# awentzonline/tartangan

Measured on AMD Instinct MI355X. Metric: images/sec (G+D step), higher is better.
Workload: dtype f32; 1 GPU; 128:3 SA-GAN cnn G+D step (R1 penalty, Adam x2, EMA), 128x128 RGB, batch 64/GPU, global batch 64; trainer=cnn, gan_config=128:3, global_batch=64, parallelism=dp1, hip_graphs=True

## Files before the change

tartangan_amd/csrc/conv.hip:

```cpp
#include <cstdlib>
#include <type_traits>
#include <utility>

#include "common.h"

namespace {

typedef float f32x16 __attribute__((ext_vector_type(16)));
typedef float f32x4 __attribute__((ext_vector_type(4)));

constexpr int CT_THREADS = 256;

template <int TH_, int TW_, int NI_>
struct Geo {
  static constexpr int TH = TH_, TW = TW_, NI = NI_, NPIX = TH_ * TW_ * NI_;
  static_assert(NPIX == 512 || NPIX == 256 || NPIX == 64, "a pixel tile is 512 / 256 pixels (waves split pixels) or 64 (waves split K)");
  static constexpr int PPW = (NPIX == 64) ? 64 : NPIX / 4;
  static_assert(TW_ % 4 == 0, "rows are staged as float4");
};
using G4 = Geo<4, 4, 16>;
using G8 = Geo<8, 8, 4>;
using G16 = Geo<16, 16, 1>;
using GX = Geo<8, 32, 1>;
using G4k = Geo<4, 4, 4>;
// ... 623 lines not shown
  auto advance = [&]() {
    xb += xstep; xbytes -= xstep;
    wb += wstep; wbytes -= wstep;
  };
  auto issue = [&](int c0, float* buf) {
    const __amdgpu_buffer_rsrc_t rx = __builtin_amdgcn_make_buffer_rsrc(const_cast<char*>(xb), 0, (int)xbytes, 0x00020000);
    const __amdgpu_buffer_rsrc_t rw = __builtin_amdgcn_make_buffer_rsrc(const_cast<char*>(wb), 0, (int)wbytes, 0x00020000);
    const int cvalid = s.Cin - c0;
#pragma unroll
    for (int i = 0; i < NPIECE; ++i) issue_piece(i, buf, rx, rw, cvalid);
    advance();
  };

  int lane_b[NT];
#pragma unroll
  for (int n = 0; n < NT; ++n) lane_b[n] = (h + g0 * KG) * P::CIS + P::pix(pix0 + n * MF + j);
  const int lane_a = DGRAD ? ((h + g0 * KG) * F::RS + j * 9 + 8) : (j * F::RS + (h + g0 * KG) * 9);

  typename Core::acc_t acc[MT][NT];
  Core::zero(acc);

#ifdef TG_DIAG_STAMPS
  asm volatile("" :: "v"(poff[0]), "v"(woff[0]), "v"(lane_b[0]), "v"(lane_a));
  const uint64_t st_setup = __builtin_amdgcn_s_memtime();
#endif
  if (DB) issue(0, lds);
  int buf = 0;
#ifdef TG_DIAG_STAMPS
  const uint64_t st_c0 = __builtin_amdgcn_s_memtime(), st_r0 = __builtin_amdgcn_s_memrealtime();
  uint64_t st_wait = 0, st_bar = 0, st_issue = 0, st_mfma = 0, st_prev = 0, st_last = 0;
#endif
  for (int c0 = 0; c0 < s.Cin; c0 += CK) {
    if constexpr (!DB) {
      __syncthreads();
      issue(c0, lds);
    }
#ifdef TG_DIAG_STAMPS
    const uint64_t ph0 = __builtin_amdgcn_s_memtime();
#endif
    asm volatile("s_waitcnt vmcnt(0)" ::: "memory");
#ifdef TG_DIAG_STAMPS
    const uint64_t ph1 = __builtin_amdgcn_s_memtime();
#endif
    __syncthreads();
#ifdef TG_DIAG_STAMPS
    const uint64_t ph2 = __builtin_amdgcn_s_memtime();
#endif
    if constexpr (DB) {
      if (c0 + CK < s.Cin) issue(c0 + CK, lds + (buf ^ 1) * BUF);
    }
#ifdef TG_DIAG_STAMPS
    const uint64_t ph3 = __builtin_amdgcn_s_memtime();
    st_wait += ph1 - ph0; st_bar += ph2 - ph1; st_issue += ph3 - ph2; st_last = ph3;
    if (c0 > 0) st_mfma += ph0 - st_prev;
    st_prev = ph3;
#endif
    const float* pl = lds + buf * BUF;
    const float* wl = pl + PBUF;
#ifdef TG_DIAG_STAMPS
    if (xcd_swizzle & 4) { buf ^= 1; continue; }
#endif
    if (prio) __builtin_amdgcn_s_setprio(0);
#pragma unroll
    for (int gi = 0; gi < NG / (WK ? 4 : 1); ++gi) {
      const int g = gi * (WK ? 4 : 1);
#pragma unroll
      for (int tap = 0; tap < 9; ++tap) {
        const int kh = tap / 3, kw = tap % 3;
        float a[MT], b[NT];
#pragma unroll
        for (int m = 0; m < MT; ++m)
          a[m] = DGRAD ? wl[lane_a + (g * KG) * F::RS + m * MF * 9 - tap] : wl[lane_a + m * MF * F::RS + (g * KG) * 9 + tap];
#pragma unroll
        for (int n = 0; n < NT; ++n) b[n] = pl[lane_b[n] + (g * KG) * P::CIS + kh * P::PWS + kw];
#pragma unroll
        for (int m = 0; m < MT; ++m)
#pragma unroll
          for (int n = 0; n < NT; ++n) {
            if constexpr (MF == 32)
              acc[m][n] = __builtin_amdgcn_mfma_f32_32x32x2f32(a[m], b[n], acc[m][n], 0, 0, 0);
            else
              acc[m][n] = __builtin_amdgcn_mfma_f32_16x16x4f32(a[m], b[n], acc[m][n], 0, 0, 0);
          }
      }
    }
    if (prio) __builtin_amdgcn_s_setprio(3);
    if (DB) buf ^= 1;
  }
#ifdef TG_DIAG_STAMPS
  {
    const uint64_t st_c1 = __builtin_amdgcn_s_memtime(), st_r1 = __builtin_amdgcn_s_memrealtime();
    const int slot = blockIdx.y * gridDim.x + blockIdx.x;
    if (threadIdx.x == 0 && slot < TG_DIAG_SLOTS) { tg_diag_stamps[2 * slot] = st_c1 - st_c0; tg_diag_stamps[2 * slot + 1] = st_r1 - st_r0; }
    st_mfma += st_c1 - st_last;
    if (lane == 0 && slot < TG_DIAG_SLOTS) {
      unsigned long long* ph = tg_diag_phases + (slot * 4 + wave) * 4;
      ph[0] = st_wait; ph[1] = st_bar; ph[2] = st_issue; ph[3] = st_mfma;
    }
  }
#endif
  if constexpr (WK) {
    __syncthreads();
    float* red = lds;
#pragma unroll
    for (int m = 0; m < MT; ++m)
#pragma unroll
      for (int n = 0; n < NT; ++n)
#pragma unroll
        for (int r = 0; r < NREG; ++r) red[(((wave * MT + m) * NT + n) * NREG + r) * 64 + lane] = acc[m][n][r];
    __syncthreads();
    constexpr int PW_ = MT * NT * NREG * 64;
#pragma unroll
    for (int m = 0; m < MT; ++m)
#pragma unroll
      for (int n = 0; n < NT; ++n)
#pragma unroll
        for (int r = 0; r < NREG; ++r) {
          const int e = ((m * NT + n) * NREG + r) * 64 + lane;
          acc[m][n][r] = (red[e] + red[PW_ + e]) + (red[2 * PW_ + e] + red[3 * PW_ + e]);
        }
  }
#ifdef TG_DIAG_STAMPS
  if ((xcd_swizzle & 2) && acc[0][0][0] != 12345.678f) return;
#endif
  Core::epilogue(acc, bias, residual, y, s, tc, co0, pix0, j, h, wave);
#ifdef TG_DIAG_STAMPS
  {
    const uint64_t e0 = __builtin_amdgcn_s_memtime();
    asm volatile("s_waitcnt vmcnt(0)" ::: "memory");
    const uint64_t e1 = __builtin_amdgcn_s_memtime();
    const int slot = blockIdx.y * gridDim.x + blockIdx.x;
    if (lane == 0 && slot < TG_DIAG_SLOTS) {
      unsigned long long* ph = tg_diag_life + (slot * 4 + wave) * 4;
      ph[0] = st_c0 - st_begin; ph[1] = e0 - st_c0; ph[2] = e1 - e0; ph[3] = st_setup - st_begin;
    }
  }
#endif
}

template <int CO, int PX>
__global__ void __launch_bounds__(256)
conv1x1_direct_kernel(const float* __restrict__ x, const float* __restrict__ w, const float* __restrict__ bias,
                      const float* __restrict__ residual, float* __restrict__ y, int Cin, int Cout, int HW, int w_so, int w_si) {
  __shared__ __attribute__((aligned(16))) float wl[1024];
  for (int e = threadIdx.x; e < Cin * CO; e += 256) {
    const int ci = e / CO, co = e - ci * CO;
    wl[e] = co < Cout ? w[co * w_so + ci * w_si] : 0.f;
  }
  __syncthreads();
  const int b = blockIdx.y;
  const int p = (blockIdx.x * 256 + threadIdx.x) * PX;
  if (p >= HW) return;
  const float* xb = x + (int64_t)b * Cin * HW + p;
  float acc[CO][PX];
#pragma unroll
  for (int co = 0; co < CO; ++co)
#pragma unroll
    for (int u = 0; u < PX; ++u) acc[co][u] = 0.f;
#pragma unroll 4
  for (int ci = 0; ci < Cin; ++ci) {
    float xv[PX];
    if (PX == 4) {
      const float4 t = *reinterpret_cast<const float4*>(xb + (int64_t)ci * HW);
      xv[0] = t.x; xv[1] = t.y; xv[2] = t.z; xv[3] = t.w;
    } else {
      xv[0] = xb[(int64_t)ci * HW];
    }
#pragma unroll
    for (int c4 = 0; c4 < CO / 4; ++c4) {
      const float4 wv = *reinterpret_cast<const float4*>(&wl[ci * CO + 4 * c4]);
      const float ww[4] = {wv.x, wv.y, wv.z, wv.w};
#pragma unroll
      for (int k = 0; k < 4; ++k)
#pragma unroll
        for (int u = 0; u < PX; ++u) acc[4 * c4 + k][u] = fmaf(ww[k], xv[u], acc[4 * c4 + k][u]);
    }
  }
  const int64_t ob = (int64_t)b * Cout * HW + p;
#pragma unroll
  for (int co = 0; co < CO; ++co) {
    if (co >= Cout) break;
    const float bv = bias ? bias[co] : 0.f;
    float o[PX];
#pragma unroll
    for (int u = 0; u < PX; ++u) o[u] = acc[co][u] + bv;
    const int64_t off = ob + (int64_t)co * HW;
    if (PX == 4) {
      if (residual) {
        const float4 r = *reinterpret_cast<const float4*>(residual + off);
        o[0] += r.x; o[1] += r.y; o[2] += r.z; o[3] += r.w;
      }
      *reinterpret_cast<float4*>(y + off) = make_float4(o[0], o[1], o[2], o[3]);
    } else {
      if (residual) o[0] += residual[off];
      y[off] = o[0];
    }
  }
}

template <int CO>
static int launch_conv1x1_direct(const float* x, const float* w, const float* bias, const float* residual, float* y, Shape s,
                                 bool dgrad, hipStream_t st) {
  const int HW = s.H * s.W;
  const int w_so = dgrad ? 1 : s.Cin, w_si = dgrad ? s.Cout : 1;
  const bool vec = (HW % 4 == 0) && tg_aligned16(x) && tg_aligned16(y) && (!residual || tg_aligned16(residual));
  if (vec) {
    dim3 grid((HW / 4 + 255) / 256, s.B);
    conv1x1_direct_kernel<CO, 4><<<grid, 256, 0, st>>>(x, w, bias, residual, y, s.Cin, s.Cout, HW, w_so, w_si);
  } else {
    dim3 grid((HW + 255) / 256, s.B);
    conv1x1_direct_kernel<CO, 1><<<grid, 256, 0, st>>>(x, w, bias, residual, y, s.Cin, s.Cout, HW, w_so, w_si);
  }
  return tg_launch_status();
}
static inline int conv1x1_co(int Cout) { return Cout <= 4 ? 4 : 8; }
static inline bool conv1x1_direct_ok(const Shape& s) { return s.Cout <= 8 && s.Cin * conv1x1_co(s.Cout) <= 1024 && s.B <= 65535; }
static int launch_conv1x1(const float* x, const float* w, const float* bias, const float* residual, float* y, Shape s, bool dgrad,
                          hipStream_t st) {
  if (s.Cout <= 4) return launch_conv1x1_direct<4>(x, w, bias, residual, y, s, dgrad, st);
  return launch_conv1x1_direct<8>(x, w, bias, residual, y, s, dgrad, st);
}

struct ChanSegs {
  float* p[3];
  int start[4];
  __device__ __forceinline__ int find(int c) const { return c >= start[2] ? 2 : (c >= start[1] ? 1 : 0); }
  __device__ __forceinline__ int width(int k) const { return start[k + 1] - start[k]; }
};
static inline ChanSegs one_seg(const float* p, int channels) {
  ChanSegs g;
  g.p[0] = g.p[1] = g.p[2] = const_cast<float*>(p);
  g.start[0] = 0; g.start[1] = g.start[2] = g.start[3] = channels;
  return g;
}
static inline ChanSegs three_segs(const float* p0, const float* p1, const float* p2, int c0, int c1, int c2) {
  ChanSegs g;
  g.p[0] = const_cast<float*>(p0); g.p[1] = const_cast<float*>(p1); g.p[2] = const_cast<float*>(p2);
  g.start[0] = 0; g.start[1] = c0; g.start[2] = c0 + c1; g.start[3] = c0 + c1 + c2;
  return g;
}

template <int NCO>
__global__ void __launch_bounds__(256)
conv1x1_mfma_kernel(ChanSegs xs, const float* __restrict__ w, const float* __restrict__ bias,
                    const float* __restrict__ residual, ChanSegs ys, int Cin, int Cout, int HW, int64_t quads,
                    int w_so, int w_si) {
  const int lane = threadIdx.x & 63, j = lane & 15, h = lane >> 4;
  const int64_t q = ((int64_t)blockIdx.x * 4 + (threadIdx.x >> 6)) * 16 + j;
  const bool live = q < quads;
  const int qpp = HW >> 2;
  const int64_t b = live ? q / qpp : 0;
  const int p = live ? (int)(q - b * qpp) * 4 : 0;
  f32x4 acc[NCO][4];
#pragma unroll
  for (int m = 0; m < NCO; ++m)
#pragma unroll
    for (int r = 0; r < 4; ++r) acc[m][r] = f32x4{0.f, 0.f, 0.f, 0.f};
  int wrow[NCO];
#pragma unroll
  for (int m = 0; m < NCO; ++m) wrow[m] = min(16 * m + j, Cout - 1) * w_so;
  constexpr int U = 4;
  for (int k0 = 0; k0 < Cin; k0 += 4 * U) {
    float4 xv[U];
    float a[U][NCO];
#pragma unroll
    for (int u = 0; u < U; ++u) {
      const int ci = k0 + 4 * u + h;
      const bool ok = live && ci < Cin;
      const int cc = min(ci, Cin - 1);
      const int k = xs.find(cc);
      const float* src = xs.p[k] + ((b * xs.width(k) + (cc - xs.start[k])) * HW + p);
      xv[u] = ok ? *reinterpret_cast<const float4*>(src) : make_float4(0.f, 0.f, 0.f, 0.f);
#pragma unroll
      for (int m = 0; m < NCO; ++m) a[u][m] = (ci < Cin) ? w[wrow[m] + cc * w_si] : 0.f;
    }
#pragma unroll
    for (int u = 0; u < U; ++u) {
      const float bx[4] = {xv[u].x, xv[u].y, xv[u].z, xv[u].w};
#pragma unroll
      for (int m = 0; m < NCO; ++m)
#pragma unroll
        for (int r = 0; r < 4; ++r) acc[m][r] = __builtin_amdgcn_mfma_f32_16x16x4f32(a[u][m], bx[r], acc[m][r], 0, 0, 0);
    }
  }
  if (!live) return;
  const float* rb = residual ? residual + (b * Cout) * HW + p : nullptr;
#pragma unroll
  for (int m = 0; m < NCO; ++m)
#pragma unroll
    for (int i = 0; i < 4; ++i) {
      const int co = 16 * m + 4 * h + i;
      if (co >= Cout) continue;
      const float bv = bias ? bias[co] : 0.f;
      float4 o = make_float4(acc[m][0][i] + bv, acc[m][1][i] + bv, acc[m][2][i] + bv, acc[m][3][i] + bv);
      if (rb) {
        const float4 t = *reinterpret_cast<const float4*>(rb + (int64_t)co * HW);
        o.x += t.x; o.y += t.y; o.z += t.z; o.w += t.w;
      }
      const int k = ys.find(co);
      *reinterpret_cast<float4*>(ys.p[k] + ((b * ys.width(k) + (co - ys.start[k])) * HW + p)) = o;
    }
}

static inline bool conv1x1_mfma_ok(const float* x, const float* residual, const float* y, const Shape& s) {
  return (s.H * s.W) % 4 == 0 && s.Cout <= 128 && tg_aligned16(x) && tg_aligned16(y) && (!residual || tg_aligned16(residual));
}
static int launch_conv1x1_segs(ChanSegs xs, const float* w, const float* bias, const float* residual, ChanSegs ys, Shape s, bool dgrad,
                               hipStream_t st) {
  const int HW = s.H * s.W;
  const int64_t quads = (int64_t)s.B * (HW / 4);
  const int w_so = dgrad ? 1 : s.Cin, w_si = dgrad ? s.Cout : 1;
  const unsigned grid = (unsigned)((quads + 63) / 64);
  const int nco = (s.Cout + 15) / 16;
#define TG_1X1(N) conv1x1_mfma_kernel<N><<<grid, 256, 0, st>>>(xs, w, bias, residual, ys, s.Cin, s.Cout, HW, quads, w_so, w_si)
  if (nco <= 1) TG_1X1(1);
  else if (nco == 2) TG_1X1(2);
  else if (nco <= 4) TG_1X1(4);
  else TG_1X1(8);
#undef TG_1X1
  return tg_launch_status();
}
static int launch_conv1x1_mfma(const float* x, const float* w, const float* bias, const float* residual, float* y, Shape s, bool dgrad,
                               hipStream_t st) {
  return launch_conv1x1_segs(one_seg(x, s.Cin), w, bias, residual, one_seg(y, s.Cout), s, dgrad, st);
}

template <int KS> struct WgCfg {
  static constexpr int CKW = (KS == 3) ? 16 : 32;
  static constexpr int KK = KS * KS;
  static constexpr int NCOL = CKW * KK;
  static constexpr int NT = (NCOL + 15) / 16;
};
constexpr int WG_GYS = 256 + 4;

template <class G, int CT>
struct GyStager {
  static constexpr int Q = G::TW / 4;
  static constexpr int ROWS_PER_CO = G::NI * G::TH;
  static constexpr int ROWS = CT * ROWS_PER_CO;
  static constexpr int NV = (ROWS * Q + CT_THREADS - 1) / CT_THREADS;
  float4 v[NV];

  __device__ __forceinline__ void load(const float* __restrict__ gy, const Shape& s, int co0, const TileCoord& tc, bool vec) {
#pragma unroll
    for (int i = 0; i < NV; ++i) {
      const int e = threadIdx.x + i * CT_THREADS;
      float4 val = make_float4(0.f, 0.f, 0.f, 0.f);
      if (e < ROWS * Q) {
        const int q = e % Q, row = e / Q;
        const int r = row % G::TH;
        const int t = row / G::TH;
        const int img = t % G::NI, co = t / G::NI;
        const int b = tc.b0 + img, hh = tc.h0 + r, ww = tc.w0 + 4 * q;
        if (b < s.B && co0 + co < s.Cout && hh < s.H && ww < s.W) {
          const float* base = gy + ((((int64_t)tc.b0 * s.Cout + co0) * s.H + tc.h0) * s.W + tc.w0);
          const float* src = base + (__umul24(__umul24(img, s.Cout) + co, s.H * s.W) + __umul24(r, s.W) + 4 * q);
          if (vec) {
            val = *reinterpret_cast<const float4*>(src);
          } else {
            val.x = src[0];
            if (ww + 1 < s.W) val.y = src[1];
            if (ww + 2 < s.W) val.z = src[2];
            if (ww + 3 < s.W) val.w = src[3];
          }
        }
      }
      v[i] = val;
    }
  }

  __device__ __forceinline__ void store(float* __restrict__ gl) const {
#pragma unroll
    for (int i = 0; i < NV; ++i) {
      const int e = threadIdx.x + i * CT_THREADS;
      if (e < ROWS * Q) {
        const int q = e % Q, row = e / Q;
        const int co = row / ROWS_PER_CO, prow = row % ROWS_PER_CO;
        *reinterpret_cast<float4*>(gl + co * WG_GYS + prow * G::TW + 4 * q) = v[i];
      }
    }
  }

  static_assert(ROWS_PER_CO * Q == 64, "one channel of a gy tile = one wave's worth of float4");
  __device__ __forceinline__ void add_channel_sums(float* acc ) const {
#pragma unroll
    for (int i = 0; i < NV; ++i) acc[i] += wave_sum((v[i].x + v[i].y) + (v[i].z + v[i].w));
  }
};

template <class G, int KS, int MTW>
__global__ void __launch_bounds__(CT_THREADS)
conv_wgrad_kernel(const float* __restrict__ x, const float* __restrict__ gy, float* __restrict__ part,
                  float* __restrict__ bias_part , Shape s, int ntiles, int S, int vec_x, int vec_gy) {
  using P = Patch<G, KS>;
  using C = WgCfg<KS>;
  constexpr int CKW = C::CKW, KK = C::KK, NT = C::NT, CT = 16 * MTW;
  constexpr int PATCH = CKW * P::CIS, GYT = CT * WG_GYS;
  constexpr int RED = 4 * MTW * NT * 4 * 64;
  constexpr int LDS_FLOATS = (PATCH + GYT) > RED ? (PATCH + GYT) : RED;
  __shared__ __attribute__((aligned(16))) float lds[LDS_FLOATS];
  float* pl = lds;
  float* gl = lds + PATCH;

  const int lane = threadIdx.x & 63, wave = threadIdx.x >> 6;
  const int j = lane & 15, h = lane >> 4;
  const int co0 = blockIdx.y * CT, ci0 = blockIdx.z * CKW;
  const int split = blockIdx.x;

  int colbase[NT];
#pragma unroll
  for (int n = 0; n < NT; ++n) {
    const int col = n * 16 + j;
    const int ci = col / KK, tap = col % KK;
    colbase[n] = (col < C::NCOL) ? (ci * P::CIS + (tap / KS) * P::PWS + (tap % KS)) : 0;
  }
  const int lane_b = pix_off<G, KS>(wave * 64) + h;
  const int lane_a = j * WG_GYS + wave * 64 + h;

  f32x4 acc[MTW][NT];
#pragma unroll
  for (int m = 0; m < MTW; ++m)
#pragma unroll
    for (int n = 0; n < NT; ++n) acc[m][n] = f32x4{0.f, 0.f, 0.f, 0.f};

  PatchStager<G, KS, CKW> ps;
  GyStager<G, CT> gs;
  const bool do_bias = (bias_part != nullptr) && (blockIdx.z == 0);
  float bsum[GyStager<G, CT>::NV];
#pragma unroll
  for (int i = 0; i < GyStager<G, CT>::NV; ++i) bsum[i] = 0.f;
  if (split < ntiles) {
    const TileCoord tc = decode_tile<G>(split, s.H, s.W);
    ps.load(x, s, s.Cin, ci0, tc, vec_x);
    gs.load(gy, s, co0, tc, vec_gy);
  }
  for (int t = split; t < ntiles; t += S) {
    __syncthreads();
    ps.store(pl);
    gs.store(gl);
    if (do_bias) gs.add_channel_sums(bsum);
    __syncthreads();
    if (t + S < ntiles) {
      const TileCoord tn = decode_tile<G>(t + S, s.H, s.W);
      ps.load(x, s, s.Cin, ci0, tn, vec_x);
      gs.load(gy, s, co0, tn, vec_gy);
    }
#pragma unroll
    for (int g = 0; g < 16; ++g) {
      constexpr int PPI = G::TH * G::TW;
      const int pg = 4 * g;
      const int goff = ((pg / PPI) * P::PH + (pg % PPI) / G::TW) * P::PWS + (pg % G::TW);
      float a[MTW], b[NT];
#pragma unroll
      for (int m = 0; m < MTW; ++m) a[m] = gl[lane_a + m * 16 * WG_GYS + 4 * g];
#pragma unroll
      for (int n = 0; n < NT; ++n) b[n] = pl[colbase[n] + lane_b + goff];
#pragma unroll
      for (int m = 0; m < MTW; ++m)
#pragma unroll
        for (int n = 0; n < NT; ++n) acc[m][n] = __builtin_amdgcn_mfma_f32_16x16x4f32(a[m], b[n], acc[m][n], 0, 0, 0);
    }
  }

  if (do_bias && lane == 0) {
#pragma unroll
    for (int i = 0; i < GyStager<G, CT>::NV; ++i) {
      const int co = co0 + 4 * i + wave;
      if (4 * i + wave < CT && co < s.Cout) bias_part[(int64_t)split * s.Cout + co] = bsum[i];
    }
  }
  __syncthreads();
  float* red = lds;
#pragma unroll
  for (int m = 0; m < MTW; ++m)
#pragma unroll
    for (int n = 0; n < NT; ++n)
#pragma unroll
      for (int r = 0; r < 4; ++r) red[(((wave * MTW + m) * NT + n) * 4 + r) * 64 + lane] = acc[m][n][r];
  __syncthreads();
  constexpr int PER_WAVE = MTW * NT * 4 * 64;
  for (int e = threadIdx.x; e < PER_WAVE; e += CT_THREADS) {
    const float v = (red[e] + red[PER_WAVE + e]) + (red[2 * PER_WAVE + e] + red[3 * PER_WAVE + e]);
    const int l = e & 63, q = e >> 6;
    const int r = q & 3, n = (q >> 2) % NT, m = (q >> 2) / NT;
    const int col = n * 16 + (l & 15);
    const int co = co0 + m * 16 + (l >> 4) * 4 + r;
    const int ci = ci0 + col / KK, tap = col % KK;
    if (col < C::NCOL && co < s.Cout && ci < s.Cin)
      part[(((int64_t)split * s.Cout + co) * s.Cin + ci) * KK + tap] = v;
  }
}

constexpr int WGD_GYQ = 65;
template <class G, int MTW, int CKW, bool DB>
__global__ void __launch_bounds__(CT_THREADS)
conv_wgrad_dma_kernel(const float* __restrict__ x, const float* __restrict__ gy, float* __restrict__ part,
                      float* __restrict__ bias_part , Shape s, int ntiles, int S) {
  static_assert(G::NPIX == 256 && WG_GYS == 4 * WGD_GYQ, "256-pixel tiles");
  using P = DPatch<G>;
  constexpr int KK = 9, CT = 16 * MTW, NCOL = CKW * KK, NT = (NCOL + 15) / 16;
  constexpr int PCH = CKW * P::CPC, GCH = CT * WGD_GYQ;
  constexpr int PCHP = dma_pad(PCH), GCHP = dma_pad(GCH);
  constexpr int NVP = (PCHP + CT_THREADS - 1) / CT_THREADS, NVG = (GCHP + CT_THREADS - 1) / CT_THREADS;
  constexpr int PBUF = PCHP * 4, BUF = PBUF + GCHP * 4;
  constexpr int RED = 4 * MTW * NT * 4 * 64 + 4 * CT;
  constexpr int LDSF = ((DB ? 2 : 1) * BUF > RED) ? (DB ? 2 : 1) * BUF : RED;
  __shared__ __attribute__((aligned(16))) float lds[LDSF];

  const int lane = threadIdx.x & 63, wave = wave_index();
  if (s.prio) __builtin_amdgcn_s_setprio(3);
  const int j = lane & 15, h = lane >> 4;
  const int co0 = blockIdx.y * CT, ci0 = blockIdx.z * CKW;
  const int split = blockIdx.x;
  const uint32_t HW = (uint32_t)(s.H * s.W);

  int colbase[NT];
#pragma unroll
  for (int n = 0; n < NT; ++n) {
    const int col = n * 16 + j;
    const int ci = col / KK, tap = col % KK;
    colbase[n] = (col < NCOL) ? (ci * P::CIS + (tap / 3) * P::PWS + (tap % 3)) : 0;
  }
  const int lane_b = P::pix(wave * 64) + h;
  const int lane_a = j * WG_GYS + wave * 64 + h;

  f32x4 acc[MTW][NT];
#pragma unroll
  for (int m = 0; m < MTW; ++m)
#pragma unroll
    for (int n = 0; n < NT; ++n) acc[m][n] = f32x4{0.f, 0.f, 0.f, 0.f};
  const bool do_bias = (bias_part != nullptr) && (blockIdx.z == 0);
  float bsum[MTW];
#pragma unroll
  for (int m = 0; m < MTW; ++m) bsum[m] = 0.f;

  const int cvalid = min(CKW, s.Cin - ci0);
  auto issue = [&](int t, float* buf) {
    const TileCoord tc = decode_tile<G>(t, s.H, s.W);
    const char* xb = reinterpret_cast<const char*>(x) + ((int64_t)tc.b0 * s.Cin + ci0) * HW * 4;
    const int64_t xbytes = ((int64_t)(s.B - tc.b0) * s.Cin - ci0) * HW * 4;
    const char* gb = reinterpret_cast<const char*>(gy) + ((int64_t)tc.b0 * s.Cout + co0) * HW * 4;
    const int64_t gbytes = ((int64_t)(s.B - tc.b0) * s.Cout - co0) * HW * 4;
    const __amdgpu_buffer_rsrc_t rx = __builtin_amdgcn_make_buffer_rsrc(const_cast<char*>(xb), 0, (int)xbytes, 0x00020000);
    const __amdgpu_buffer_rsrc_t rg = __builtin_amdgcn_make_buffer_rsrc(const_cast<char*>(gb), 0, (int)gbytes, 0x00020000);
#pragma unroll
    for (int i = 0; i < NVP; ++i) {
      const int e = i * CT_THREADS + threadIdx.x;
      const int ci = e / P::CPC, rem = e % P::CPC;
      const int row = rem / P::QR, q = rem % P::QR;
      const int img = row / P::PH, r = row % P::PH;
      const int hh = tc.h0 + r - 1, ww = tc.w0 - 4 + 4 * q;
      const bool ok = (rem < P::RAW / 4) && (ci < cvalid) && (tc.b0 + img < s.B) && (hh >= 0) && (hh < s.H) && (ww >= 0) && (ww < s.W);
      const uint32_t off = ok ? (__umul24(__umul24(img, s.Cin) + ci, HW) + __umul24(hh, s.W) + ww) << 2 : DMA_OOB;
      if ((i + 1) * CT_THREADS <= PCHP || i * CT_THREADS + wave * 64 < PCHP) dma16(rx, buf + (i * CT_THREADS + wave * 64) * 4, off);
    }
#pragma unroll
    for (int i = 0; i < NVG; ++i) {
      const int e = i * CT_THREADS + threadIdx.x;
      const int co = e / WGD_GYQ, q = e % WGD_GYQ;
      const int p = 4 * q;
      const int img = p / (G::TH * G::TW), rem = p % (G::TH * G::TW);
      const int hh = tc.h0 + rem / G::TW, ww = tc.w0 + rem % G::TW;
      const bool ok = (e < GCH) && (q < 64) && (co0 + co < s.Cout) && (tc.b0 + img < s.B) && (hh < s.H) && (ww < s.W);
      const uint32_t off = ok ? (__umul24(__umul24(img, s.Cout) + co, HW) + __umul24(hh, s.W) + ww) << 2 : DMA_OOB;
      if ((i + 1) * CT_THREADS <= GCHP || i * CT_THREADS + wave * 64 < GCHP) dma16(rg, buf + PBUF + (i * CT_THREADS + wave * 64) * 4, off);
    }
  };
  auto compute = [&](const float* buf) {
    const float* pl = buf;
    const float* gl = buf + PBUF;
    if (s.prio) __builtin_amdgcn_s_setprio(0);
#pragma unroll
    for (int g = 0; g < 16; ++g) {
      constexpr int PPI = G::TH * G::TW;
      const int pg = 4 * g;
      const int goff = ((pg / PPI) * P::PH + (pg % PPI) / G::TW) * P::PWS + (pg % G::TW);
      float a[MTW], b[NT];
#pragma unroll
      for (int m = 0; m < MTW; ++m) a[m] = gl[lane_a + m * 16 * WG_GYS + 4 * g];
#pragma unroll
      for (int n = 0; n < NT; ++n) b[n] = pl[colbase[n] + lane_b + goff];
#pragma unroll
      for (int m = 0; m < MTW; ++m) bsum[m] += a[m];
#pragma unroll
      for (int m = 0; m < MTW; ++m)
#pragma unroll
        for (int n = 0; n < NT; ++n) acc[m][n] = __builtin_amdgcn_mfma_f32_16x16x4f32(a[m], b[n], acc[m][n], 0, 0, 0);
    }
    if (s.prio) __builtin_amdgcn_s_setprio(3);
  };

  if constexpr (DB) {
    if (split < ntiles) issue(split, lds);
    int buf = 0;
    for (int t = split; t < ntiles; t += S) {
      asm volatile("s_waitcnt vmcnt(0)" ::: "memory");
      __syncthreads();
      if (t + S < ntiles) issue(t + S, lds + (buf ^ 1) * BUF);
      compute(lds + buf * BUF);
      buf ^= 1;
    }
  } else {
    for (int t = split; t < ntiles; t += S) {
      __syncthreads();
      issue(t, lds);
      asm volatile("s_waitcnt vmcnt(0)" ::: "memory");
      __syncthreads();
      compute(lds);
    }
  }

  __syncthreads();
  float* red = lds;
#pragma unroll
  for (int m = 0; m < MTW; ++m)
#pragma unroll
    for (int n = 0; n < NT; ++n)
#pragma unroll
      for (int r = 0; r < 4; ++r) red[(((wave * MTW + m) * NT + n) * 4 + r) * 64 + lane] = acc[m][n][r];
  constexpr int PER_WAVE = MTW * NT * 4 * 64;
  float* bred = lds + 4 * PER_WAVE;
  if (do_bias) {
#pragma unroll
    for (int m = 0; m < MTW; ++m) {
      float v = bsum[m];
      v += __shfl_xor(v, 16, 64);
      v += __shfl_xor(v, 32, 64);
      if (h == 0) bred[wave * CT + m * 16 + j] = v;
    }
  }
  __syncthreads();
  for (int e = threadIdx.x; e < PER_WAVE; e += CT_THREADS) {
    const float v = (red[e] + red[PER_WAVE + e]) + (red[2 * PER_WAVE + e] + red[3 * PER_WAVE + e]);
    const int l = e & 63, q = e >> 6;
    const int r = q & 3, n = (q >> 2) % NT, m = (q >> 2) / NT;
    const int col = n * 16 + (l & 15);
    const int co = co0 + m * 16 + (l >> 4) * 4 + r;
    const int ci = ci0 + col / KK, tap = col % KK;
    if (col < NCOL && co < s.Cout && ci < s.Cin)
      part[(((int64_t)split * s.Cout + co) * s.Cin + ci) * KK + tap] = v;
  }
  if (do_bias && threadIdx.x < CT && co0 + (int)threadIdx.x < s.Cout) {
    const int c = threadIdx.x;
    bias_part[(int64_t)split * s.Cout + co0 + c] = (bred[c] + bred[CT + c]) + (bred[2 * CT + c] + bred[3 * CT + c]);
  }
}

template <int MT, int NT>
__global__ void __launch_bounds__(256)
conv1x1_wgrad_stream_kernel(const float* __restrict__ x, ChanSegs gys, float* __restrict__ part,
                            float* __restrict__ bias_part , int Cin, int Cout, int HW, int64_t groups, int S) {
  __shared__ float red[4 * MT * NT * 4 * 64 + 4 * 16 * MT];
  const int lane = threadIdx.x & 63, wave = threadIdx.x >> 6, j = lane & 15, h = lane >> 4;
  const int co0 = blockIdx.y * 16 * MT, ci0 = blockIdx.z * 16 * NT, split = blockIdx.x;
  const int64_t g_begin = groups * split / S, g_end = groups * (split + 1) / S;
  const int64_t n = g_end - g_begin;
  const int64_t w_begin = g_begin + n * wave / 4, w_end = g_begin + n * (wave + 1) / 4;
  const int gpp = HW >> 4;
  int64_t arow[MT], brow[NT], aimg[MT];
  const float* abase[MT];
#pragma unroll
  for (int m = 0; m < MT; ++m) {
    const int co = min(co0 + 16 * m + j, Cout - 1), k = gys.find(co);
    abase[m] = gys.p[k];
    aimg[m] = (int64_t)gys.width(k) * HW;
    arow[m] = (int64_t)(co - gys.start[k]) * HW + 4 * h;
  }
#pragma unroll
  for (int t = 0; t < NT; ++t) brow[t] = (int64_t)min(ci0 + 16 * t + j, Cin - 1) * HW + 4 * h;
  f32x4 acc[MT][NT];
#pragma unroll
  for (int m = 0; m < MT; ++m)
#pragma unroll
    for (int t = 0; t < NT; ++t) acc[m][t] = f32x4{0.f, 0.f, 0.f, 0.f};
  float bsum[MT];
#pragma unroll
  for (int m = 0; m < MT; ++m) bsum[m] = 0.f;
  constexpr int U = 4;
  for (int64_t g0 = w_begin; g0 < w_end; g0 += U) {
    float4 ga[U][MT], xb[U][NT];
#pragma unroll
    for (int u = 0; u < U; ++u) {
      const int64_t g = g0 + u;
      const bool ok = g < w_end;
      const int64_t b = ok ? g / gpp : 0;
      const int64_t p = ok ? (g - b * gpp) * 16 : 0;
#pragma unroll
      for (int m = 0; m < MT; ++m)
        ga[u][m] = ok ? *reinterpret_cast<const float4*>(abase[m] + b * aimg[m] + arow[m] + p) : make_float4(0.f, 0.f, 0.f, 0.f);
#pragma unroll
      for (int t = 0; t < NT; ++t)
        xb[u][t] = ok ? *reinterpret_cast<const float4*>(x + b * Cin * HW + brow[t] + p) : make_float4(0.f, 0.f, 0.f, 0.f);
    }
#pragma unroll
    for (int u = 0; u < U; ++u) {
#pragma unroll
      for (int m = 0; m < MT; ++m) bsum[m] += (ga[u][m].x + ga[u][m].y) + (ga[u][m].z + ga[u][m].w);
#pragma unroll
      for (int m = 0; m < MT; ++m) {
        const float av[4] = {ga[u][m].x, ga[u][m].y, ga[u][m].z, ga[u][m].w};
#pragma unroll
        for (int t = 0; t < NT; ++t) {
          const float bv[4] = {xb[u][t].x, xb[u][t].y, xb[u][t].z, xb[u][t].w};
#pragma unroll
          for (int r = 0; r < 4; ++r) acc[m][t] = __builtin_amdgcn_mfma_f32_16x16x4f32(av[r], bv[r], acc[m][t], 0, 0, 0);
        }
      }
    }
  }
  constexpr int PER_WAVE = MT * NT * 4 * 64;
#pragma unroll
  for (int m = 0; m < MT; ++m)
#pragma unroll
    for (int t = 0; t < NT; ++t)
#pragma unroll
      for (int i = 0; i < 4; ++i) red[wave * PER_WAVE + ((m * NT + t) * 4 + i) * 64 + lane] = acc[m][t][i];
  float* bred = red + 4 * PER_WAVE;
  const bool do_bias = bias_part != nullptr && blockIdx.z == 0;
  if (do_bias) {
#pragma unroll
    for (int m = 0; m < MT; ++m) {
      float v = bsum[m];
      v += __shfl_xor(v, 16, 64);
      v += __shfl_xor(v, 32, 64);
      if (h == 0) bred[wave * 16 * MT + 16 * m + j] = v;
    }
  }
  __syncthreads();
  for (int e = threadIdx.x; e < PER_WAVE; e += 256) {
    const float v = (red[e] + red[PER_WAVE + e]) + (red[2 * PER_WAVE + e] + red[3 * PER_WAVE + e]);
    const int l = e & 63, q = e >> 6;
    const int i = q & 3, t = (q >> 2) % NT, m = (q >> 2) / NT;
    const int co = co0 + 16 * m + 4 * (l >> 4) + i, ci = ci0 + 16 * t + (l & 15);
    if (co < Cout && ci < Cin) part[((int64_t)split * Cout + co) * Cin + ci] = v;
  }
  if (do_bias && threadIdx.x < 16 * MT && co0 + (int)threadIdx.x < Cout) {
    const int c = threadIdx.x;
    bias_part[(int64_t)split * Cout + co0 + c] = (bred[c] + bred[16 * MT + c]) + (bred[2 * 16 * MT + c] + bred[3 * 16 * MT + c]);
  }
}

static int conv1x1_mode();
static inline bool conv1x1_wgrad_stream_ok(const float* x, const float* gy, const Shape& s) {
  return conv1x1_mode() != 0 && (s.H * s.W) % 16 == 0 && tg_aligned16(x) && tg_aligned16(gy);
}
static int launch_conv1x1_wgrad_segs(const float* x, ChanSegs gy, float* part, float* bias_part, Shape s, int S, hipStream_t st) {
  const int HW = s.H * s.W;
  const int64_t groups = (int64_t)s.B * (HW / 16);
  const int mt = s.Cout > 16 ? 2 : 1, nt = s.Cin > 16 ? 2 : 1;
  dim3 grid(S, (s.Cout + 16 * mt - 1) / (16 * mt), (s.Cin + 16 * nt - 1) / (16 * nt));
  if (mt == 1 && nt == 1) conv1x1_wgrad_stream_kernel<1, 1><<<grid, 256, 0, st>>>(x, gy, part, bias_part, s.Cin, s.Cout, HW, groups, S);
  else if (mt == 1) conv1x1_wgrad_stream_kernel<1, 2><<<grid, 256, 0, st>>>(x, gy, part, bias_part, s.Cin, s.Cout, HW, groups, S);
  else if (nt == 1) conv1x1_wgrad_stream_kernel<2, 1><<<grid, 256, 0, st>>>(x, gy, part, bias_part, s.Cin, s.Cout, HW, groups, S);
  else conv1x1_wgrad_stream_kernel<2, 2><<<grid, 256, 0, st>>>(x, gy, part, bias_part, s.Cin, s.Cout, HW, groups, S);
  return tg_launch_status();
}
static int launch_conv1x1_wgrad_stream(const float* x, const float* gy, float* part, float* bias_part, Shape s, int S, hipStream_t st) {
  return launch_conv1x1_wgrad_segs(x, one_seg(gy, s.Cout), part, bias_part, s, S, st);
}

__device__ __forceinline__ void wgrad_reduce_block(int blk, const float* __restrict__ part, float* __restrict__ gw, int64_t E, int S,
                                                   const float* __restrict__ bias_part, float* __restrict__ gbias, int Cout,
                                                   int accumulate) {
  __shared__ float red[4][64];
  const int lane = threadIdx.x & 63, wave = threadIdx.x >> 6;
  const int eblocks = (int)((E + 63) / 64);
  const float* src = part;
  float* dst = gw;
  int64_t n = E, e = blk * 64ll + lane;
  if (blk >= eblocks) {
    src = bias_part; dst = gbias; n = Cout;
    e = (blk - eblocks) * 64ll + lane;
  }
  float a0 = 0.f, a1 = 0.f, a2 = 0.f, a3 = 0.f;
  if (e < n) {
    int sidx = wave;
    for (; sidx + 12 < S; sidx += 16) {
      a0 += src[(int64_t)sidx * n + e];
      a1 += src[(int64_t)(sidx + 4) * n + e];
      a2 += src[(int64_t)(sidx + 8) * n + e];
      a3 += src[(int64_t)(sidx + 12) * n + e];
    }
    for (; sidx < S; sidx += 4) a0 += src[(int64_t)sidx * n + e];
  }
  red[wave][lane] = (a0 + a1) + (a2 + a3);
  __syncthreads();
  if (wave == 0 && e < n) {
    const float r = (red[0][lane] + red[1][lane]) + (red[2][lane] + red[3][lane]);
    dst[e] = accumulate ? dst[e] + r : r;
  }
}

__global__ void __launch_bounds__(256) wgrad_reduce_kernel(const float* __restrict__ part, float* __restrict__ gw, int64_t E, int S,
                                                           const float* __restrict__ bias_part, float* __restrict__ gbias, int Cout,
                                                           int accumulate) {
  wgrad_reduce_block(blockIdx.x, part, gw, E, S, bias_part, gbias, Cout, accumulate);
}

constexpr int RB_MAX_ITEMS = 40;
struct ReduceItem {
  const float* part; float* gw; float* gbias;
  int64_t E;
  int S, Cout, accumulate, pad;
};
struct ReduceBatch {
  int n;
  int block_end[RB_MAX_ITEMS];
  ReduceItem item[RB_MAX_ITEMS];
};
__global__ void __launch_bounds__(256) wgrad_reduce_batch_kernel(ReduceBatch rb) {
  int i = 0;
  while (i + 1 < rb.n && (int)blockIdx.x >= rb.block_end[i]) ++i;
  const ReduceItem it = rb.item[i];
  const int blk = blockIdx.x - (i > 0 ? rb.block_end[i - 1] : 0);
  wgrad_reduce_block(blk, it.part, it.gw, it.E, it.S, it.gbias ? it.part + (int64_t)it.S * it.E : nullptr, it.gbias, it.Cout,
                     it.accumulate);
}

__global__ void __launch_bounds__(256) upconv_weights_kernel(const float* __restrict__ w, float* __restrict__ wp, int n ) {
  const int e = blockIdx.x * 256 + threadIdx.x;
  if (e >= n) return;
  float k[3][3];
#pragma unroll
  for (int i = 0; i < 9; ++i) k[i / 3][i % 3] = w[(int64_t)e * 9 + i];
#pragma unroll
  for (int dy = 0; dy < 2; ++dy)
#pragma unroll
    for (int dx = 0; dx < 2; ++dx) {
      float r[2][3];
#pragma unroll
      for (int c = 0; c < 3; ++c) {
        r[0][c] = dy == 0 ? k[0][c] : k[0][c] + k[1][c];
        r[1][c] = dy == 0 ? k[1][c] + k[2][c] : k[2][c];
      }
      float* o = wp + ((int64_t)(dy * 2 + dx) * n + e) * 4;
#pragma unroll
      for (int ty = 0; ty < 2; ++ty) {
        o[ty * 2 + 0] = dx == 0 ? r[ty][0] : r[ty][0] + r[ty][1];
        o[ty * 2 + 1] = dx == 0 ? r[ty][1] + r[ty][2] : r[ty][2];
      }
    }
}

template <class G, bool WK>
__global__ void __launch_bounds__(CT_THREADS)
conv_upfwd_kernel(const float* __restrict__ x, const float* __restrict__ wp, const float* __restrict__ bias,
                  const float* __restrict__ residual, float* __restrict__ y, Shape s, int vec_x, int vec_w) {
  constexpr int KS = 2, CT = 16, NT = 4, KG = 4;
  using P = Patch<G, KS>;
  using WT = WTile<KS, CT, WK>;
  constexpr int KK = WT::KK, CK = WT::CK, CTS = WT::CTS, NG = CK / KG, GSTEP = WK ? 4 : 1;
  static_assert(G::NPIX == (WK ? 64 : 256) && KK == 4 && NG % GSTEP == 0, "256-pixel tiles (or 64, K split over the waves), 2x2 windows");
  constexpr int STAGE = CK * P::CIS + 4 * WT::SIZE, REDF = WK ? 4 * 2 * NT * 4 * 64 : 0;
  __shared__ __attribute__((aligned(16))) float lds[STAGE > REDF ? STAGE : REDF];
  float* pl = lds;
  float* wl = lds + CK * P::CIS;
  const int lane = threadIdx.x & 63, wave = threadIdx.x >> 6;
  const int j = lane & 15, h = lane >> 4;
  const TileCoord tc = decode_tile<G>(blockIdx.x, s.H, s.W);
  const int co0 = blockIdx.y * CT;
  const int pix0 = WK ? 0 : wave * 64;
  const int k0 = WK ? wave * KG : 0;
  int lane_b[NT];
#pragma unroll
  for (int n = 0; n < NT; ++n) lane_b[n] = (h + k0) * P::CIS + pix_off<G, KS>(pix0 + n * 16 + j);
  const int lane_a = ((h + k0) * KK) * CTS + j;
  f32x4 acc[4][NT];
#pragma unroll
  for (int ph = 0; ph < 4; ++ph)
#pragma unroll
    for (int n = 0; n < NT; ++n) acc[ph][n] = f32x4{0.f, 0.f, 0.f, 0.f};

  PatchStager<G, KS, CK> ps;
  WeightStager<KS, CT, false, WK> ws[4];
  const size_t phase_stride = (size_t)s.Cout * s.Cin * KK;
  ps.load(x, s, s.Cin, 0, tc, vec_x);
#pragma unroll
  for (int ph = 0; ph < 4; ++ph) ws[ph].load(wp + ph * phase_stride, s.Cin, s.Cout, 0, co0, vec_w);
  for (int ci0 = 0; ci0 < s.Cin; ci0 += CK) {
    __syncthreads();
    ps.store(pl);
#pragma unroll
    for (int ph = 0; ph < 4; ++ph) ws[ph].store(wl + ph * WT::SIZE);
    __syncthreads();
    if (ci0 + CK < s.Cin) {
      ps.load(x, s, s.Cin, ci0 + CK, tc, vec_x);
#pragma unroll
      for (int ph = 0; ph < 4; ++ph) ws[ph].load(wp + ph * phase_stride, s.Cin, s.Cout, ci0 + CK, co0, vec_w);
    }
#pragma unroll
    for (int gi = 0; gi < NG / GSTEP; ++gi) {
      const int g = gi * GSTEP;
#pragma unroll
      for (int kh = 0; kh < 3; ++kh)
#pragma unroll
        for (int kw = 0; kw < 3; ++kw) {
          float b[NT];
#pragma unroll
          for (int n = 0; n < NT; ++n) b[n] = pl[lane_b[n] + (g * KG) * P::CIS + kh * P::PWS + kw];
#pragma unroll
          for (int dy = 0; dy < 2; ++dy)
#pragma unroll
            for (int dx = 0; dx < 2; ++dx) {
              const int ty = kh - dy, tx = kw - dx;
              if (ty < 0 || ty > 1 || tx < 0 || tx > 1) continue;
              const float a = wl[(dy * 2 + dx) * WT::SIZE + lane_a + ((g * KG) * KK + ty * 2 + tx) * CTS];
#pragma unroll
              for (int n = 0; n < NT; ++n)
                acc[dy * 2 + dx][n] = __builtin_amdgcn_mfma_f32_16x16x4f32(a, b[n], acc[dy * 2 + dx][n], 0, 0, 0);
            }
        }
    }
  }

  if constexpr (WK) {
    float* red = lds;
    constexpr int PW_ = 2 * NT * 4 * 64;
#pragma unroll
    for (int dy = 0; dy < 2; ++dy) {
      __syncthreads();
#pragma unroll
      for (int dx = 0; dx < 2; ++dx)
#pragma unroll
        for (int n = 0; n < NT; ++n)
#pragma unroll
          for (int r = 0; r < 4; ++r) red[wave * PW_ + ((dx * NT + n) * 4 + r) * 64 + lane] = acc[dy * 2 + dx][n][r];
      __syncthreads();
#pragma unroll
      for (int n = 0; n < NT; ++n) {
        if (n != wave) continue;
#pragma unroll
        for (int dx = 0; dx < 2; ++dx)
#pragma unroll
          for (int r = 0; r < 4; ++r) {
            const int e = ((dx * NT + n) * 4 + r) * 64 + lane;
            acc[dy * 2 + dx][n][r] = (red[e] + red[PW_ + e]) + (red[2 * PW_ + e] + red[3 * PW_ + e]);
          }
      }
    }
  }

  const int W2 = 2 * s.W;
  const uint32_t HW2 = (uint32_t)(2 * s.H * W2);
  const int64_t tile0 = ((((int64_t)tc.b0 * s.Cout + co0) * (2 * s.H) + 2 * tc.h0) * W2 + 2 * tc.w0) * 4;
  char* ybase = reinterpret_cast<char*>(y) + tile0;
  const char* rbase = reinterpret_cast<const char*>(residual) + tile0;
  float bv[4];
#pragma unroll
  for (int r = 0; r < 4; ++r) bv[r] = bias ? bias[min(co0 + 4 * h + r, s.Cout - 1)] : 0.f;
#pragma unroll
  for (int n = 0; n < NT; ++n) {
    if (WK && n != wave) continue;
    const int p = pix0 + n * 16 + j;
    const int img = p / (G::TH * G::TW), rem = p % (G::TH * G::TW);
    const int pr = rem / G::TW, pc = rem % G::TW;
    if (tc.b0 + img >= s.B || tc.h0 + pr >= s.H || tc.w0 + pc >= s.W) continue;
    const uint32_t lane_off = __umul24(__umul24(img, s.Cout) + 4 * h, HW2) + __umul24(2 * pr, W2) + 2 * pc;
#pragma unroll
    for (int r = 0; r < 4; ++r) {
      if (co0 + 4 * h + r >= s.Cout) continue;
#pragma unroll
      for (int dy = 0; dy < 2; ++dy) {
        const uint32_t off = (lane_off + (uint32_t)r * HW2 + (uint32_t)(dy * W2)) << 2;
        float2 o = make_float2(acc[dy * 2][n][r] + bv[r], acc[dy * 2 + 1][n][r] + bv[r]);
        if (residual) {
          const float2 rr = *reinterpret_cast<const float2*>(rbase + off);
          o.x += rr.x; o.y += rr.y;
        }
        *reinterpret_cast<float2*>(ybase + off) = o;
      }
    }
  }
}

__global__ void __launch_bounds__(256) upconvT_weights_kernel(const float* __restrict__ w, float* __restrict__ w4t, int Cout, int Cin) {
  const int e = blockIdx.x * 256 + threadIdx.x;
  if (e >= Cout * Cin) return;
  const int ci = e / Cout, co = e - ci * Cout;
  float k[3][3];
#pragma unroll
  for (int i = 0; i < 9; ++i) k[i / 3][i % 3] = w[((int64_t)co * Cin + ci) * 9 + i];
  float r[4][3];
#pragma unroll
  for (int c = 0; c < 3; ++c) { r[0][c] = k[2][c]; r[1][c] = k[1][c] + k[2][c]; r[2][c] = k[0][c] + k[1][c]; r[3][c] = k[0][c]; }
  float* o = w4t + (int64_t)e * 16;
#pragma unroll
  for (int u = 0; u < 4; ++u) { o[u * 4 + 0] = r[u][2]; o[u * 4 + 1] = r[u][1] + r[u][2]; o[u * 4 + 2] = r[u][0] + r[u][1]; o[u * 4 + 3] = r[u][0]; }
}

__global__ void __launch_bounds__(256) upconv_weights_pair_kernel(const float* __restrict__ w, float* __restrict__ wp, float* __restrict__ w4t,
                                                                  int Cout, int Cin) {
  const int e = blockIdx.x * 256 + threadIdx.x;
  const int n = Cout * Cin;
  if (e >= n) return;
  const int co = e / Cin, ci = e - co * Cin;
  float k[3][3];
#pragma unroll
  for (int i = 0; i < 9; ++i) k[i / 3][i % 3] = w[(int64_t)e * 9 + i];
#pragma unroll
  for (int dy = 0; dy < 2; ++dy)
#pragma unroll
    for (int dx = 0; dx < 2; ++dx) {
      float r[2][3];
#pragma unroll
      for (int c = 0; c < 3; ++c) {
        r[0][c] = dy == 0 ? k[0][c] : k[0][c] + k[1][c];
        r[1][c] = dy == 0 ? k[1][c] + k[2][c] : k[2][c];
      }
      float* o = wp + ((int64_t)(dy * 2 + dx) * n + e) * 4;
#pragma unroll
      for (int ty = 0; ty < 2; ++ty) {
        o[ty * 2 + 0] = dx == 0 ? r[ty][0] : r[ty][0] + r[ty][1];
        o[ty * 2 + 1] = dx == 0 ? r[ty][1] + r[ty][2] : r[ty][2];
      }
    }
  float r[4][3];
#pragma unroll
  for (int c = 0; c < 3; ++c) { r[0][c] = k[2][c]; r[1][c] = k[1][c] + k[2][c]; r[2][c] = k[0][c] + k[1][c]; r[3][c] = k[0][c]; }
  float* o = w4t + ((int64_t)ci * Cout + co) * 16;
#pragma unroll
  for (int u = 0; u < 4; ++u) { o[u * 4 + 0] = r[u][2]; o[u * 4 + 1] = r[u][1] + r[u][2]; o[u * 4 + 2] = r[u][0] + r[u][1]; o[u * 4 + 3] = r[u][0]; }
}

template <class G>
struct Patch2x {
  static constexpr int PH = 2 * G::TH + 2, TW2 = 2 * G::TW;
  static constexpr int IOFF = 4, ORG = IOFF - 1;
  static constexpr int PWS = TW2 + 2 * IOFF;
  static constexpr int IMG = PH * PWS;
  static constexpr int RAW = G::NI * IMG;
  static constexpr int CIS = ((RAW + 31) / 32) * 32 + 16;
  static constexpr int PPI = G::TH * G::TW;
  static_assert(PPI % 64 == 0, "a wave's 64 pixels stay inside one image");
  __device__ __forceinline__ static int pix(int p) {
    const int img = p / PPI, rem = p % PPI;
    return img * IMG + 2 * (rem / G::TW) * PWS + 2 * (rem % G::TW) + ORG;
  }
};

template <class G, int CK>
struct PatchStager2x {
  using P = Patch2x<G>;
  static constexpr int Q = P::TW2 / 4;
  static constexpr int ROWS = CK * G::NI * P::PH;
  static constexpr int NV = (ROWS * Q + CT_THREADS - 1) / CT_THREADS;
  static constexpr int NHALO = ROWS * 2;
  static constexpr int NH = (NHALO + CT_THREADS - 1) / CT_THREADS;
  float4 v[NV];
  float hv[NH];
  __device__ __forceinline__ void load(const float* __restrict__ gy, int B, int C, int H2, int W2, int c0, const TileCoord& tc, bool vec) {
    const char* base = reinterpret_cast<const char*>(gy) + ((((int64_t)tc.b0 * C + c0) * H2 + (2 * tc.h0 - 1)) * W2 + (2 * tc.w0 - 1)) * 4;
    const uint32_t HW2 = (uint32_t)(H2 * W2);
#pragma unroll
    for (int i = 0; i < NV; ++i) {
      const int e = threadIdx.x + i * CT_THREADS;
      float4 val = make_float4(0.f, 0.f, 0.f, 0.f);
      if (e < ROWS * Q) {
// ... 1660 lines not shown
```

Baseline: 6986 images/s.

## Add LDS-staged pipelined 1x1 conv kernel and double-buffer the 1x1 wgrad loop

Adds a new 1x1 conv forward/dgrad kernel that stages the weight slice in shared memory, splits output channels across a second grid dimension when the pixel grid is small, and prefetches input channel groups with a triple-buffered register pipeline. It also double-buffers the 1x1 wgrad streaming loads for the smaller tile shapes so loads for the next block overlap MFMA work on the current one. The aim is to hide global-memory latency and raise occupancy on small-spatial layers. The cost is extra shared memory and register pressure, and an env var keeps the legacy path selectable.

```diff
diff --git a/tartangan_amd/csrc/conv.hip b/tartangan_amd/csrc/conv.hip
--- a/tartangan_amd/csrc/conv.hip
+++ b/tartangan_amd/csrc/conv.hip
@@ -949,6 +949,112 @@
     }
 }
 
+template <int NCO>
+__global__ void __launch_bounds__(256)
+conv1x1_mfma_stream_kernel(ChanSegs xs, const float* __restrict__ w, const float* __restrict__ bias,
+                           const float* __restrict__ residual, ChanSegs ys, int Cin, int Cout, int HW, int64_t quads,
+                           int w_so, int w_si) {
+  extern __shared__ __attribute__((aligned(16))) float wl1[];
+  constexpr int U = 4, NB = 3, CB = 16 * NCO, HEAD = 8;
+  const int lane = threadIdx.x & 63, j = lane & 15, h = lane >> 4;
+  const int64_t q = ((int64_t)blockIdx.x * 4 + (threadIdx.x >> 6)) * 16 + j;
+  const bool live = q < quads;
+  const int qpp = HW >> 2;
+  const int64_t b = live ? q / qpp : 0;
+  const int p = live ? (int)(q - b * qpp) * 4 : 0;
+  const int G = (Cin + 15) >> 4;
+  const int co0 = blockIdx.y * CB;
+  const int total = G * 16 * CB;
+  auto fetch = [&](int e, int& slot) -> float {
+    int col, ci;
+    if (w_si == 1) { const int t = e >> 4; col = t % CB; ci = (t / CB) * 16 + (e & 15); }
+    else { col = e % CB; ci = e / CB; }
+    slot = (ci * 16 + (col & 15)) * NCO + (col >> 4);
+    return ci < Cin ? w[min(co0 + col, Cout - 1) * w_so + ci * w_si] : 0.f;
+  };
+  auto load_group = [&](float4 (&dst)[U], int g) {
+#pragma unroll
+    for (int u = 0; u < U; ++u) {
+      const int ci = 16 * g + 4 * u + h;
+      const bool ok = live && ci < Cin;
+      const int cc = min(ci, Cin - 1);
+      const int k = xs.find(cc);
+      const float* src = xs.p[k] + ((b * xs.width(k) + (cc - xs.start[k])) * HW + p);
+      dst[u] = ok ? *reinterpret_cast<const float4*>(src) : make_float4(0.f, 0.f, 0.f, 0.f);
+    }
+  };
+  for (int e = HEAD * 256 + threadIdx.x; e < total; e += 256) {
+    int slot;
+    const float v = fetch(e, slot);
+    wl1[slot] = v;
+  }
+  float wr[HEAD];
+  int ws[HEAD];
+#pragma unroll
+  for (int i = 0; i < HEAD; ++i) {
+    const int e = i * 256 + threadIdx.x;
+    ws[i] = -1;
+    wr[i] = 0.f;
+    if (e < total) wr[i] = fetch(e, ws[i]);
+  }
+  float4 xv[NB][U];
+#pragma unroll
+  for (int s = 0; s < NB - 1; ++s)
+    if (s < G) load_group(xv[s], s);
+#pragma unroll
+  for (int i = 0; i < HEAD; ++i)
+    if (ws[i] >= 0) wl1[ws[i]] = wr[i];
+  __syncthreads();
+  f32x4 acc[NCO][4];
+#pragma unroll
+  for (int m = 0; m < NCO; ++m)
+#pragma unroll
+    for (int r = 0; r < 4; ++r) acc[m][r] = f32x4{0.f, 0.f, 0.f, 0.f};
+  for (int g0 = 0; g0 < G; g0 += NB) {
+#pragma unroll
+    for (int s = 0; s < NB; ++s) {
+      const int g = g0 + s;
+      if (g < G) {
+        if (g + NB - 1 < G) load_group(xv[(s + NB - 1) % NB], g + NB - 1);
+#pragma unroll
+        for (int u = 0; u < U; ++u) {
+          const float* ap = wl1 + ((16 * g + 4 * u + h) * 16 + j) * NCO;
+          float a[NCO];
+#pragma unroll
+          for (int m = 0; m < NCO; ++m) a[m] = ap[m];
+          const float bx[4] = {xv[s][u].x, xv[s][u].y, xv[s][u].z, xv[s][u].w};
+#pragma unroll
+          for (int m = 0; m < NCO; ++m)
+#pragma unroll
+            for (int r = 0; r < 4; ++r) acc[m][r] = __builtin_amdgcn_mfma_f32_16x16x4f32(a[m], bx[r], acc[m][r], 0, 0, 0);
+        }
+      }
+    }
+  }
+  if (!live) return;
+  const float* rb = residual ? residual + (b * Cout) * HW + p : nullptr;
+#pragma unroll
+  for (int m = 0; m < NCO; ++m)
+#pragma unroll
+    for (int i = 0; i < 4; ++i) {
+      const int co = co0 + 16 * m + 4 * h + i;
+      if (co >= Cout) continue;
+      const float bv = bias ? bias[co] : 0.f;
+      float4 o = make_float4(acc[m][0][i] + bv, acc[m][1][i] + bv, acc[m][2][i] + bv, acc[m][3][i] + bv);
+      if (rb) {
+        const float4 t = *reinterpret_cast<const float4*>(rb + (int64_t)co * HW);
+        o.x += t.x; o.y += t.y; o.z += t.z; o.w += t.w;
+      }
+      const int k = ys.find(co);
+      *reinterpret_cast<float4*>(ys.p[k] + ((b * ys.width(k) + (co - ys.start[k])) * HW + p)) = o;
+    }
+}
+
+static int conv1x1_legacy() {
+  static const int v = [] { const char* e = getenv("TG_CONV1X1_LEGACY"); return e ? atoi(e) : 0; }();
+  return v;
+}
+
 static inline bool conv1x1_mfma_ok(const float* x, const float* residual, const float* y, const Shape& s) {
   return (s.H * s.W) % 4 == 0 && s.Cout <= 128 && tg_aligned16(x) && tg_aligned16(y) && (!residual || tg_aligned16(residual));
 }
@@ -959,6 +1065,21 @@
   const int w_so = dgrad ? 1 : s.Cin, w_si = dgrad ? s.Cout : 1;
   const unsigned grid = (unsigned)((quads + 63) / 64);
   const int nco = (s.Cout + 15) / 16;
+  if (!conv1x1_legacy() && grid <= 16 * 256) {
+    int per = nco <= 1 ? 1 : nco == 2 ? 2 : nco <= 4 ? 4 : 8;
+    while (per > 1 && (int64_t)grid * ((nco + per - 1) / per) < 512) per >>= 1;
+    const size_t lds = (size_t)((s.Cin + 15) / 16) * 256 * per * sizeof(float);
+    if (lds <= 32768) {
+      const dim3 g2(grid, (nco + per - 1) / per);
+#define TG_1X1S(N) conv1x1_mfma_stream_kernel<N><<<g2, 256, lds, st>>>(xs, w, bias, residual, ys, s.Cin, s.Cout, HW, quads, w_so, w_si)
+      if (per == 1) TG_1X1S(1);
+      else if (per == 2) TG_1X1S(2);
+      else if (per == 4) TG_1X1S(4);
+      else TG_1X1S(8);
+#undef TG_1X1S
+      return tg_launch_status();
+    }
+  }
 #define TG_1X1(N) conv1x1_mfma_kernel<N><<<grid, 256, 0, st>>>(xs, w, bias, residual, ys, s.Cin, s.Cout, HW, quads, w_so, w_si)
   if (nco <= 1) TG_1X1(1);
   else if (nco == 2) TG_1X1(2);
@@ -1293,7 +1414,7 @@
   }
 }
 
-template <int MT, int NT>
+template <int MT, int NT, bool PIPE>
 __global__ void __launch_bounds__(256)
 conv1x1_wgrad_stream_kernel(const float* __restrict__ x, ChanSegs gys, float* __restrict__ part,
                             float* __restrict__ bias_part , int Cin, int Cout, int HW, int64_t groups, int S) {
@@ -1324,8 +1445,8 @@
 #pragma unroll
   for (int m = 0; m < MT; ++m) bsum[m] = 0.f;
   constexpr int U = 4;
-  for (int64_t g0 = w_begin; g0 < w_end; g0 += U) {
-    float4 ga[U][MT], xb[U][NT];
+  struct Block { float4 ga[U][MT], xb[U][NT]; };
+  auto load_block = [&](Block& k, int64_t g0) {
 #pragma unroll
     for (int u = 0; u < U; ++u) {
       const int64_t g = g0 + u;
@@ -1334,11 +1455,15 @@
       const int64_t p = ok ? (g - b * gpp) * 16 : 0;
 #pragma unroll
       for (int m = 0; m < MT; ++m)
-        ga[u][m] = ok ? *reinterpret_cast<const float4*>(abase[m] + b * aimg[m] + arow[m] + p) : make_float4(0.f, 0.f, 0.f, 0.f);
+        k.ga[u][m] = ok ? *reinterpret_cast<const float4*>(abase[m] + b * aimg[m] + arow[m] + p) : make_float4(0.f, 0.f, 0.f, 0.f);
 #pragma unroll
       for (int t = 0; t < NT; ++t)
-        xb[u][t] = ok ? *reinterpret_cast<const float4*>(x + b * Cin * HW + brow[t] + p) : make_float4(0.f, 0.f, 0.f, 0.f);
-    }
+        k.xb[u][t] = ok ? *reinterpret_cast<const float4*>(x + b * Cin * HW + brow[t] + p) : make_float4(0.f, 0.f, 0.f, 0.f);
+    }
+  };
+  auto use_block = [&](const Block& k) {
+    const auto& ga = k.ga;
+    const auto& xb = k.xb;
 #pragma unroll
     for (int u = 0; u < U; ++u) {
 #pragma unroll
@@ -1351,6 +1476,26 @@
           const float bv[4] = {xb[u][t].x, xb[u][t].y, xb[u][t].z, xb[u][t].w};
 #pragma unroll
           for (int r = 0; r < 4; ++r) acc[m][t] = __builtin_amdgcn_mfma_f32_16x16x4f32(av[r], bv[r], acc[m][t], 0, 0, 0);
+        }
+      }
+    }
+  };
+  if constexpr (!PIPE) {
+    for (int64_t g0 = w_begin; g0 < w_end; g0 += U) {
+      Block k;
+      load_block(k, g0);
+      use_block(k);
+    }
+  } else {
+    Block k[2];
+    if (w_begin < w_end) load_block(k[0], w_begin);
+    for (int64_t g0 = w_begin; g0 < w_end; g0 += 2 * U) {
+#pragma unroll
+      for (int s = 0; s < 2; ++s) {
+        const int64_t gs = g0 + s * U;
+        if (gs < w_end) {
+          if (gs + U < w_end) load_block(k[1 - s], gs + U);
+          use_block(k[s]);
         }
       }
     }
@@ -1396,10 +1541,19 @@
   const int64_t groups = (int64_t)s.B * (HW / 16);
   const int mt = s.Cout > 16 ? 2 : 1, nt = s.Cin > 16 ? 2 : 1;
   dim3 grid(S, (s.Cout + 16 * mt - 1) / (16 * mt), (s.Cin + 16 * nt - 1) / (16 * nt));
-  if (mt == 1 && nt == 1) conv1x1_wgrad_stream_kernel<1, 1><<<grid, 256, 0, st>>>(x, gy, part, bias_part, s.Cin, s.Cout, HW, groups, S);
-  else if (mt == 1) conv1x1_wgrad_stream_kernel<1, 2><<<grid, 256, 0, st>>>(x, gy, part, bias_part, s.Cin, s.Cout, HW, groups, S);
-  else if (nt == 1) conv1x1_wgrad_stream_kernel<2, 1><<<grid, 256, 0, st>>>(x, gy, part, bias_part, s.Cin, s.Cout, HW, groups, S);
-  else conv1x1_wgrad_stream_kernel<2, 2><<<grid, 256, 0, st>>>(x, gy, part, bias_part, s.Cin, s.Cout, HW, groups, S);
+#define TG_WG1X1(M, N, P) conv1x1_wgrad_stream_kernel<M, N, P><<<grid, 256, 0, st>>>(x, gy, part, bias_part, s.Cin, s.Cout, HW, groups, S)
+  if (conv1x1_legacy()) {
+    if (mt == 1 && nt == 1) TG_WG1X1(1, 1, false);
+    else if (mt == 1) TG_WG1X1(1, 2, false);
+    else if (nt == 1) TG_WG1X1(2, 1, false);
+    else TG_WG1X1(2, 2, false);
+  } else {
+    if (mt == 1 && nt == 1) TG_WG1X1(1, 1, true);
+    else if (mt == 1) TG_WG1X1(1, 2, true);
+    else if (nt == 1) TG_WG1X1(2, 1, true);
+    else TG_WG1X1(2, 2, false);
+  }
+#undef TG_WG1X1
   return tg_launch_status();
 }
 static int launch_conv1x1_wgrad_stream(const float* x, const float* gy, float* part, float* bias_part, Shape s, int S, hipStream_t st) {
```

Measured after the change: 7038 images/s (median of 6 runs). No clear change (+0.7%).
